# exosports/transit

Hardware: AMD Instinct MI355X
Metric: wavenumber-points*layers/sec (CH4 2-4um emission spectrum) (higher is better)
Workload: dtype f64; 1 GPU; BASELINE configs[1]: CH4-demo-shaped emission: 2500-5000 cm-1 @1 cm-1, wnosamp 2160, CH4 lines, eclipse, 5 angles, H2-H2 CIA; n_wn=2501, n_layers=100, layers_needed=81, n_lines=1000000, parallelism=one GPU

## Files before the change

transit_amd/csrc/hip/trx_api.hip:

```cpp
#include <hip/hip_runtime.h>
#include <rccl/rccl.h>
#include <dlfcn.h>
#include <functional>

#include <algorithm>
#include <chrono>
#include <cmath>
#include <cstdio>
#include <cstdlib>
#include <cstring>
#include <atomic>
#include <condition_variable>
#include <memory>
#include <mutex>
#include <string>
#include <thread>
#include <vector>

#include "transit_hip.h"
#include "trx_kernels.hip.h"
#include "trx_walk.hip.h"
#include "trx_rows.hip.h"
#include "trx_tail.hip.h"
#include "trx_lanes.hip.h"
// ... 9 lines not shown
  void release() { if (p) { (void)hipFree(p); p = nullptr; bytes = 0; } }
  template <class T> T *as() const { return (T *)p; }
};

struct DevView {
  void *p = nullptr;
  template <class T> T *as() const { return (T *)p; }
};

}

struct trx_handle {
  int device = 0;
  hipStream_t stream = nullptr, stream2 = nullptr;
  hipStream_t stream4 = nullptr;
  std::vector<hipEvent_t> ev_ac, ev_cb;
  hipEvent_t ev_walk1 = nullptr;
  hipEvent_t ev_inputs = nullptr, ev_cia = nullptr, ev_join = nullptr, ev_run_a = nullptr, ev_run_b = nullptr;
  std::string err;

  double wn_i = 0, wn_d = 0, odwn = 0; int64_t nwn = 0, nown = 0, lo = 0, hi = 0, nsh = 0; int osamp = 1;
  int niso = 0, nmol = 0;
  std::vector<double> iso_mass, iso_ratio, mol_mass, mol_radius, mol_pol;
  std::vector<double> pair_csd, pair_sqrt;
  std::vector<int32_t> iso_imol, mol_is_h2;
  std::vector<double> iso_wmin, iso_wmax;
  int ndop = 0, nlor = 0;
  std::vector<double> adop, alor;
  std::vector<int32_t> psizeT; bool psize_mono = false;
  std::vector<double> dopthr;
  std::vector<double> lorthr;
  std::vector<int> guess_dop, guess_lor, guess_a0, guess_a1;
  std::vector<long> guess_npre;
  std::vector<double> iso_sqrtm;
  std::vector<double> dens_over_m;
  std::vector<int32_t> psize; std::vector<long long> poff; int64_t tab_n = 0;
  DevBuf d_adop, d_dopthr, d_e2tab, d_psize, d_poff, d_tab, d_tabT, d_poffT, d_gimod, d_gidiv;
  float *tab = nullptr; const float *tabT = nullptr; const long long *poffT = nullptr;
  DevBuf d_tabW, d_walkprof; const float *tabW = nullptr; bool tabw_ok = false;
  DevBuf d_tabW32, d_wp32; const float *tabW32 = nullptr; unsigned slab32 = 0;
  long long row_m8_from = 768;
  std::vector<std::pair<double, double>> recip_ok;
  bool shard_frames = true;
  bool cia_window = true;
  bool cia_sums = true;
  bool cia_segments = true;
  bool two_queues = true;
  bool tail_direct = true;
  bool ray_tail = true;
  bool packed_walk = true; int packed_max_layers = 10;
  bool no_binrec = false;
  int xcd_map = 1;
  bool lanes_walk = true, lanes_force = false; int max_gcount = 0; DevBuf d_linebase, d_rinfo;
  bool no_row_copy = false, no_rows32 = false;
  bool row_staging = true;
  int64_t nlines = 0, ngroups = 0, nadd = 0, ninrange = 0;
  DevBuf d_lgroup, d_wavn, d_elow, d_gf, d_iso, d_inr, d_gfirst, d_gcount, d_giown, d_giso, d_gwavn, d_gblock, d_cntge, d_cntsub;
  int sub_f = 1;
  LinesDev L{};
  HostBuf<double> h_gwavn; std::vector<int32_t> h_gblock; HostBuf<int32_t> h_cntge, h_gfirst, h_gcount;
  void *comm = nullptr; int nranks = 1, rank = 0;
  bool windowed() const { return lo > 0 || hi < nwn; }
  DevBuf d_cand, d_candrec; int64_t ncand = -1;
  DevBuf d_kmax;
  int kmax_parity = 0, kmax_nr = 0; bool kmax_clean = false;
  DevBuf d_walk, d_wbase, d_part[2];
  std::vector<int32_t> h_wbase; int nwaves = 0, ngw = 0; bool walk_ok = false;
  bool walk_temp_ok = true;
  struct Plan { bool built = false; DevBuf blo, bhi, off, binw, binrec; int64_t records = 0; };
  Plan plan[4];
  struct Cia { int nspec; int mol[2]; std::vector<double> wn, temp, cs, zt, uw, ruw, rh, wf, wb; DevBuf d_wn, d_temp, d_cs, d_zt, d_uw, d_ruw, d_rh, d_wf, d_wb; };
  std::vector<Cia> cia;
  DevBuf d_cia_ws;
  int ws_nr = 0, ws_chunk = 0;
  DevBuf d_SG, d_idop8, d_sticky, d_part3;
  DevBuf d_in; void *h_in = nullptr; size_t h_in_bytes = 0; const double *h_in_dev = nullptr;
  DevBuf d_pm_f64, d_pm_i32;
  DevBuf d_xf;
  DevBuf d_small; DevView d_flags, d_status, d_counters; void *h_small = nullptr; size_t h_small_bytes = 0;
  DevBuf d_e, d_ecs, d_er, d_tau, d_last, d_intens, d_spec, d_acc, d_geom;
  bool has_grid = false; long og_nmol = 0, og_ntemp = 0, og_nlayer = 0, og_nwave = 0;
  std::vector<double> og_temp; std::vector<int32_t> og_molidx; DevBuf d_og_o, d_og_layer, d_og_itemp, d_iso_mx, d_pm, d_kmaxpm;
  trx_stats stats{};
  std::vector<double> run_f64, run_geom, run_ipv; std::vector<int32_t> run_i32;
  int hint_layers = 0;
  DevBuf d_e_saved; std::vector<uint8_t> saved;
  void *h_spec = nullptr; size_t h_spec_bytes = 0;
  void *h_spec_dev = nullptr, *h_small_dev = nullptr;
  void *h_tailblk = nullptr, *h_tailblk_dev = nullptr; size_t h_tailblk_bytes = 0;
};

namespace {

struct LogSink { trx_log_fn fn = nullptr; void *user = nullptr; int max_level = 0; };
LogSink &log_sink() { static LogSink s; return s; }
void log_msg(int level, const std::string &msg)
{
  const LogSink s = log_sink();
  if (s.fn && level <= s.max_level) s.fn(level, msg.c_str(), s.user);
}

struct StageTimer {
  std::chrono::steady_clock::time_point t = std::chrono::steady_clock::now();
  void lap(const char *what) {
    const auto n = std::chrono::steady_clock::now();
    if (log_sink().fn && log_sink().max_level >= TRX_LOG_DEBUG) {
// ... 77 lines not shown
  logspace((double)s->lmin, (double)s->lmax, nl, h->alor);
  h->psize.assign((size_t)nd * nl, 0); h->poff.assign((size_t)nd * nl, 0);
  const double dwn = s->wn_d / s->osamp;
  int64_t total = 0, bins = 0;
  for (int i = 0; i < nd; i++)
    for (int j = 0; j < nl; j++) {
      const size_t k = (size_t)i * nl + j;
      if (h->adop[i] * 10.0 < h->alor[j] && i != 0) {
        h->psize[k] = h->psize[k - nl]; h->poff[k] = h->poff[k - nl];
        continue;
      }
      const float dop = (float)h->adop[i], lor = (float)h->alor[j];
      double big = dop; if (big < lor) big = lor;
      const double wv = big * s->timesalpha;
      int nv = 2 * (long)(wv / dwn + 0.5) + 1;
      if (nv < 2) nv = 3;
      if (nv > 2 * (int)s->nown) nv = 2 * (int)s->nown + 1;
      if (nv < 0) return fail(h, TRX_E_ARG, "negative Voigt profile size");
      ProfileJob J{};
      J.off = total; J.nv = nv; J.alphaL = lor; J.alphaD = dop;
      J.half = dwn * (long)(nv / 2);
      const bool quick = nv > 99999;
      double step = 2.0 * J.half / (nv - 1);
      int npts = 50; double sub = J.alphaD / (npts - 1);
      if (step < sub || quick) { sub = step; J.regime = quick ? 0 : 1; J.m = 1; }
      else {
        npts = (int)(step / sub) + 1;
        if (npts & 1) npts++;
        J.m = npts; J.regime = 2;
        const long long tot = (long long)nv * npts + 1;
        if (tot > 2000000000LL) return fail(h, TRX_E_UNSUPPORTED, "Voigt sub-sampling exceeds int range");
        sub = 2.0 * J.half / (double)(tot - 1);
      }
      J.sub = sub; J.first_bin = bins;
      jobs.push_back(J);
      h->psize[k] = nv / 2; h->poff[k] = total;
      total += nv; bins += nv;
    }
  h->tab_n = total;
  return TRX_OK;
}

void test_switches(trx_handle *h)
{
  h->no_row_copy = std::getenv("TRX_NO_ROW_COPY") != nullptr;
  h->no_rows32 = std::getenv("TRX_NO_ROWS32") != nullptr;
  h->row_staging = !std::getenv("TRX_NO_ROW_STAGING");
  if (const char *v = std::getenv("TRX_ROWS_M8_FROM")) h->row_m8_from = std::atoll(v);
  h->packed_walk = !std::getenv("TRX_NO_PACKED_WALK");
  if (const char *v = std::getenv("TRX_PACKED_MAX_LAYERS")) h->packed_max_layers = std::max(1, std::min(32, std::atoi(v)));
  if (const char *e = std::getenv("TRX_XCD_MAP")) h->xcd_map = std::atoi(e);
  h->no_binrec = std::getenv("TRX_NO_BINREC") != nullptr;
  if (const char *e = std::getenv("TRX_LANES_WALK")) { h->lanes_walk = std::atoi(e) != 0; h->lanes_force = std::atoi(e) == 2; }
  if (const char *e = std::getenv("TRX_RAY_TAIL")) h->ray_tail = std::atoi(e) != 0;
  if (const char *e = std::getenv("TRX_CIA_SUMS")) h->cia_sums = std::atoi(e) != 0;
  if (const char *e = std::getenv("TRX_CIA_SEGMENTS")) h->cia_segments = std::atoi(e) != 0;
  if (const char *e = std::getenv("TRX_TWO_QUEUES")) h->two_queues = std::atoi(e) != 0;
  if (const char *e = std::getenv("TRX_TAIL_DIRECT")) h->tail_direct = std::atoi(e) != 0;
  if (const char *e = std::getenv("TRX_CIA_WINDOW")) h->cia_window = std::atoi(e) != 0;
  if (const char *e = std::getenv("TRX_SHARD_FRAMES")) h->shard_frames = std::atoi(e) != 0;
}

int build_table(trx_handle *h, const trx_static *s)
{
  std::vector<ProfileJob> jobs;
  int rc = plan_table(h, s, jobs);
  if (rc) return rc;
  double coef[64]; long double fact = 1.0L;
  for (int n = 0; n < 64; n++) { if (n > 0) fact *= (long double)n; coef[n] = (double)(1.0L / (fact * (long double)(2 * n + 1))); }
  HIPCHK(h, hipMemcpyToSymbolAsync(HIP_SYMBOL(c_voigt_coef), coef, sizeof(coef), 0, hipMemcpyHostToDevice, h->stream));
  DevBuf d_jobs;
  if ((rc = upload(h, d_jobs, jobs))) return rc;
  const size_t tab_alloc = (size_t)h->tab_n + 2 * kTabPad + (size_t)kWalkMaxFrame * (size_t)std::min<int64_t>(s->osamp, 1 << 21) + kRowTail;
  if ((rc = ensure(h, h->d_tab, sizeof(float) * tab_alloc))) return rc;
  HIPCHK(h, hipMemsetAsync(h->d_tab.p, 0, sizeof(float) * tab_alloc, h->stream));
  h->tab = h->d_tab.as<float>() + kTabPad;
  std::vector<int32_t> ps32(h->psize.begin(), h->psize.end());
  if ((rc = upload(h, h->d_psize, ps32))) return rc;
  if ((rc = upload(h, h->d_poff, h->poff))) return rc;
  if ((rc = upload(h, h->d_adop, h->adop))) return rc;
  {
    const int nd = s->ndop;
    std::vector<double> thr((size_t)nd + 1);
    thr[0] = -HUGE_VAL; thr[nd] = HUGE_VAL;
    auto idx = [&](double v) { return nearest_index(h->adop.data(), v, 0, nd); };
    for (int k = 1; k < nd; k++) {
      uint64_t a, b; double x;
      std::memcpy(&a, &h->adop[k - 1], 8); std::memcpy(&b, &h->adop[k], 8);
      while (b - a > 1) {
        const uint64_t m = a + (b - a) / 2;
        std::memcpy(&x, &m, 8);
        if (idx(x) >= k) b = m; else a = m;
      }
      std::memcpy(&thr[k], &b, 8);
      if (idx(thr[k]) != k || idx(std::nextafter(thr[k], 0.0)) != k - 1)
        return fail(h, TRX_E_ARG, "Doppler-width grid is not strictly increasing");
    }
    if ((rc = upload(h, h->d_dopthr, thr))) return rc;
    h->dopthr = thr;
    {
      const int nl = s->nlor;
      std::vector<double> lt((size_t)nl + 1);
      lt[0] = -HUGE_VAL; lt[nl] = HUGE_VAL;
      auto lidx = [&](double v) { return nearest_index(h->alor.data(), v, 0, nl); };
      bool ok = true;
      for (int k = 1; k < nl && ok; k++) {
// ... 59 lines not shown
                         d_joffT.as<long long>() + j0, h->tab, h->d_tabT.as<float>() + kTabPad, s->osamp, 0);
    }
    HIPCHK(h, hipStreamSynchronize(h->stream));
    h->tabT = h->d_tabT.as<float>() + kTabPad; h->poffT = h->d_poffT.as<long long>();
  }
  {
    std::vector<long long> joffW(jobs.size());
    long long totW = 0;
    for (size_t j = 0; j < jobs.size(); j++) {
      int front, stride; walk_row_layout((jobs[j].nv - 1) / s->osamp + 1, front, stride);
      joffW[j] = totW; totW += (long long)s->osamp * stride;
    }
    test_switches(h);
    h->tabw_ok = 4 * (totW + 2 * (long long)kTabPad) < (1LL << 32) && !h->no_row_copy;
    if (h->tabw_ok) {
      std::vector<WalkProfile> desc((size_t)s->ndop * s->nlor);
      size_t j = 0;
      for (int i = 0; i < s->ndop; i++)
        for (int k = 0; k < s->nlor; k++) {
          const size_t e = (size_t)i * s->nlor + k;
          if (h->adop[i] * 10.0 < h->alor[k] && i != 0) { desc[e] = desc[e - s->nlor]; continue; }
          const long long ps = h->psize[e], K = (2 * ps) / s->osamp + 1;
          int front, stride; walk_row_layout((int)K, front, stride);
          desc[e].centre4 = (uint32_t)(4 * (joffW[j++] + front + ps / s->osamp));
          desc[e].rowb = (int32_t)(4 * stride);
          desc[e].psr = (int32_t)(ps % s->osamp);
          desc[e].ps = (int32_t)ps;
        }
      DevBuf d_joffW;
      if ((rc = upload(h, d_joffW, joffW)) || (rc = upload(h, h->d_walkprof, desc))) return rc;
      if ((rc = ensure(h, h->d_tabW, sizeof(float) * ((size_t)totW + 2 * kTabPad)))) return rc;
      HIPCHK(h, hipMemsetAsync(h->d_tabW.p, 0, sizeof(float) * ((size_t)totW + 2 * kTabPad), h->stream));
      for (size_t j0 = 0; j0 < jobs.size(); j0 += 32768) {
        const int nj = (int)std::min<size_t>(32768, jobs.size() - j0);
        hipLaunchKernelGGL(k_table_phase_major, dim3(32, nj), dim3(256), 0, h->stream, d_jobs.as<ProfileJob>() + j0,
                           d_joffW.as<long long>() + j0, h->tab, h->d_tabW.as<float>() + kTabPad, s->osamp, 1);
      }
      {
        std::vector<long long> joff32(jobs.size(), -1);
        std::vector<uint32_t> c32((size_t)s->ndop * s->nlor, 0xffffffffu);
        long long nq = 0; size_t jj = 0;
        for (int i = 0; i < s->ndop; i++)
          for (int k = 0; k < s->nlor; k++) {
            const size_t e = (size_t)i * s->nlor + k;
            if (h->adop[i] * 10.0 < h->alor[k] && i != 0) { c32[e] = c32[e - s->nlor]; continue; }
            const long long ps = h->psize[e], K = (2 * ps) / s->osamp + 1;
            if (K <= 8) { joff32[jj] = 8 * nq; c32[e] = (uint32_t)(32 * nq); nq++; }
            jj++;
          }
        const long long tot32 = nq * 8 * (long long)s->osamp;
        if (nq > 0 && 32 * nq < (1LL << 24) && s->osamp < (1 << 24) && 4 * tot32 < (1LL << 32) && !h->no_rows32) {
          DevBuf d_joff32;
          if ((rc = upload(h, d_joff32, joff32)) || (rc = upload(h, h->d_wp32, c32))) return rc;
          if ((rc = ensure(h, h->d_tabW32, sizeof(float) * (size_t)tot32))) return rc;
          for (size_t j0 = 0; j0 < jobs.size(); j0 += 32768) {
            const int nj = (int)std::min<size_t>(32768, jobs.size() - j0);
            hipLaunchKernelGGL(k_table_rows32, dim3(16, nj), dim3(256), 0, h->stream, d_jobs.as<ProfileJob>() + j0,
                               d_joffW.as<long long>() + j0, d_joff32.as<long long>() + j0, h->d_tabW.as<float>() + kTabPad, h->d_tabW32.as<float>(), s->osamp, 8 * nq);
          }
          h->slab32 = (unsigned)(32 * nq);
          HIPCHK(h, hipStreamSynchronize(h->stream));
          h->tabW32 = h->d_tabW32.as<float>();
        }
      }
      HIPCHK(h, hipStreamSynchronize(h->stream));
      h->tabW = h->d_tabW.as<float>() + kTabPad;
    }
  }
  HIPCHK(h, hipGetLastError());
  HIPCHK(h, hipEventRecord(e1, h->stream));
  HIPCHK(h, hipStreamSynchronize(h->stream));
  float ms = 0; HIPCHK(h, hipEventElapsedTime(&ms, e0, e1));
  (void)hipEventDestroy(e0); (void)hipEventDestroy(e1);
  h->stats.ms_create_table = ms;
  h->stats.table_floats = h->tab_n;
  return TRX_OK;
}

int prepare_lines(trx_handle *h, const trx_static *s)
{
  const int64_t n = s->nlines;
  StageTimer T;
  const int nth = create_threads();
  const double wn0 = s->wn_i, odwn = s->wn_d / s->osamp;
  const double own_last = wn0 + (double)(s->nown - 1) * odwn;
  if (n > 2000000000LL) return fail(h, TRX_E_UNSUPPORTED, "more than 2^31 lines per handle");
  const double *elow = s->elow, *gf = s->gf;
  int rc_raw = TRX_OK;
  std::thread raw_up([&]() {
    (void)hipSetDevice(h->device);
    if ((rc_raw = upload_raw(h, h->d_elow, elow, (size_t)n)) || (rc_raw = upload_raw(h, h->d_gf, gf, (size_t)n)) ||
        (rc_raw = upload_raw(h, h->d_iso, s->isoid, (size_t)n))) return;
  });
  struct Joiner { std::thread &t; ~Joiner() { if (t.joinable()) t.join(); } } raw_join{raw_up};
  HostBuf<double> wavn; wavn.alloc((size_t)n);
  HostBuf<uint8_t> inr; inr.alloc((size_t)n);
  {
    std::vector<int64_t> cnt((size_t)nth + 1, 0); std::vector<int> bad((size_t)nth + 1, 0);
    parallel_parts(n, nth, [&](int t, int64_t i0, int64_t i1) {
      int64_t c = 0;
      for (int64_t i = i0; i < i1; i++) {
        if (s->isoid[i] < 0 || s->isoid[i] >= s->niso) { bad[t] = 1; continue; }
        wavn[i] = 1.0 / (s->wl_um[i] * kTliWfct);
        inr[i] = !(wavn[i] < wn0 || wavn[i] > own_last);
        c += inr[i];
      }
      cnt[t] = c;
// ... 617 lines not shown
  if (!M.permol) { h->stats.walk_steps++; h->stats.walk_records += pl->records; h->stats.walk_record_lanes += pl->records * nc; }
  const size_t pbytes = sizeof(double) * kWalkLayers * (size_t)std::max<int64_t>(pl->records, 1);
  if (part.bytes < pbytes) {
    HIPCHK(h, hipStreamSynchronize(st));
    HIPCHK(h, hipStreamSynchronize(h->stream4));
    if ((rc = ensure(h, part, pbytes))) return rc;
  }
  if (ev_reuse) HIPCHK(h, hipStreamWaitEvent(st, ev_reuse, 0));
  WalkArgs A{};
  A.lines = h->d_walk.as<WalkLine>(); A.rinfo = h->d_rinfo.as<RangeInfo>(); A.gfirst = h->d_gfirst.as<int32_t>(); A.gcount = h->d_gcount.as<int32_t>();
  A.gblock = h->d_gblock.as<int32_t>(); A.P = P;
  A.niso = h->niso; A.nlor = h->nlor; A.ndop = h->ndop; A.osamp = h->osamp; A.lo = h->lo; A.hi = h->hi;
  A.r_top = r_top; A.nc = nc; A.Y = Y; A.wcut = d_wcut; A.kmax = M.d_kmax; A.ethresh = M.ethresh;
  A.nmx = M.nmx; A.iso_mx = M.d_iso_mx; A.permol = M.permol; A.sticky_idop = M.d_sticky;
  A.dthr = h->d_dopthr.as<double>(); A.e2tab = h->d_e2tab.as<double>();
  A.psize = h->d_psize.as<int32_t>(); A.poff = h->d_poff.as<long long>();
  A.table = h->tab; A.zero_index = h->tab_n;
  A.tabw = h->tabW; A.walkprof = h->d_walkprof.as<WalkProfile>();
  A.tabw32 = h->tabW32; A.wp32 = h->tabW32 ? h->d_wp32.as<uint32_t>() : nullptr; A.slab32 = h->slab32;
  A.xcd_map = h->xcd_map & 2;
  A.part = part.as<double>(); A.counters = M.prof ? h->d_counters.as<unsigned long long>() : nullptr;
  A.flags = h->d_flags.as<int>(); A.last = M.skip_done ? h->d_last.as<int>() : nullptr; A.eager = M.eager;
  unsigned nw = (unsigned)h->nwaves;
  A.nseg = 0;
  if (h->windowed() && h->niso <= kWalkSegs && nw > 0) {
    const int Rc = nb / 2 - 1;
    const long long klo = std::max<long long>(0, h->lo - Rc - 1), khi = std::min<long long>(h->nwn - 1, h->hi - 1 + Rc);
    int cum = 0, ns = 0;
    for (int b = 0; b < h->niso; b++) {
      const int gb0 = h->h_gblock[b], gb1 = h->h_gblock[b + 1];
      if (gb0 == gb1) continue;
      const int32_t *cg = &h->h_cntge[(size_t)b * (h->nwn + 1)];
      const int ga = cg[khi + 1], gz = h->lo - Rc - 1 <= 0 ? gb1 - gb0 : cg[klo];
      const int wa = h->h_wbase[b] + ga / h->ngw, wz = h->h_wbase[b] + (gz + h->ngw - 1) / h->ngw;
      if (wz <= wa) continue;
      A.seg_w0[ns] = wa; A.seg_cum[ns] = cum; cum += wz - wa; ns++;
    }
    A.seg_cum[ns] = cum; A.nseg = ns;
    nw = (unsigned)cum;
    if (ns == 0) { A.nseg = 1; A.seg_w0[0] = 0; A.seg_cum[0] = 0; A.seg_cum[1] = 0; }
  }
  const bool lanes_prod = nw > 0 && A.tabw != nullptr && nb >= 8 && nc <= kLanesMaxLayers && h->lanes_walk &&
                          h->max_gcount <= kLanesMaxGroup && (h->ngroups >= 8 * h->nwn || h->lanes_force);
  const bool packed_prod = !lanes_prod && nw > 0 && A.tabw != nullptr && nc <= h->packed_max_layers && h->packed_walk;
  const bool lanes = lanes_prod && !M.prof, packed = packed_prod && !M.prof;
  const int form_prod = lanes_prod ? 1 : packed_prod ? 2 : 0, form = lanes ? 1 : packed ? 2 : 0;
  if (form_out) *form_out = form_prod;
  if (!M.permol) { h->stats.walk_form_steps[form_prod]++; h->stats.walk_form_layers[form_prod] += nc; h->stats.walk_form_record_lanes[form_prod] += pl->records * nc; }
  if (sp && sp->begin(form == 1 ? Spans::kWalkLanes : form == 2 ? Spans::kWalkPacked : Spans::kWalk, st)) return fail(h, TRX_E_HIP, "event");
  if (lanes) {
    LanesExtra X{h->d_linebase.as<double>()};
    A.xcd_map = h->xcd_map & 1;
    if (log_sink().fn && log_sink().max_level >= TRX_LOG_DEBUG)
      log_msg(TRX_LOG_DEBUG, "walk: lanes = lines, " + std::to_string(nc) + " layers, " + std::to_string(nb) + "-bin frames");
    const dim3 grid((nw + kLanesWaves - 1) / kLanesWaves), block(64 * kLanesWaves);
    const size_t lds = lanes_lds_bytes(nc, h->ndop);
    if (nb == 8) hipLaunchKernelGGL((k_line_walk_lanes<8, 5>), grid, block, lds, st, A, X);
    else         hipLaunchKernelGGL((k_line_walk_lanes<16, 2>), grid, block, lds, st, A, X);
  }
  else if (packed) {
    const int S = 64 / nc;
    const unsigned pw = (nw + (unsigned)S - 1) / (unsigned)S;
    const dim3 grid((pw + kWalkWaves - 1) / kWalkWaves), block(64 * kWalkWaves);
    if (nb <= 4)      hipLaunchKernelGGL(k_line_walk_packed<4>, grid, block, 0, st, A, S);
    else if (nb == 8) hipLaunchKernelGGL(k_line_walk_packed<8>, grid, block, 0, st, A, S);
    else              hipLaunchKernelGGL(k_line_walk_packed<16>, grid, block, 0, st, A, S);
  }
  else if (nw > 0) {
    const bool per_bin = M.prof || (nb >= kWalkRowsFrom && A.tabw == nullptr);
    if (nb == 2) launch_walk<2>(A, per_bin, nw, st);
    else if (nb == 4) launch_walk<4>(A, per_bin, nw, st);
    else if (nb == 8) launch_walk<8>(A, per_bin, nw, st);
    else launch_walk<16>(A, per_bin, nw, st);
  }
  if (sp && sp->end(st)) return fail(h, TRX_E_HIP, "event");
  PendingCombine pc;
  pc.valid = true; pc.sc = st_comb ? st_comb : st; pc.st_walk = st; pc.cross = st_comb != nullptr && ev_walk != nullptr;
  pc.ev_walk = ev_walk; pc.ev_done = ev_done;
  if (pc.cross) HIPCHK(h, hipEventRecord(ev_walk, st));
  CombineArgs &C = pc.C;
  C.P = P; C.niso = h->niso; C.gblock = h->d_gblock.as<int32_t>(); C.lo = h->lo; C.nsh = h->nsh; C.r_top = r_top; C.nc = nc;
  C.nmx = M.nmx; C.iso_mx = M.d_iso_mx; C.part = part.as<double>(); C.e = M.d_e;
  C.flags = h->d_flags.as<int>(); C.last = A.last; C.eager = M.eager;
  if (defer) { *defer = pc; return TRX_OK; }
  return launch_combine(h, pc, sp);
}

int sweep_chunk(trx_handle *h, const LayerDev &Y, const double *d_wcut, const int32_t *psmax,
                int r_top, int nc, int nc_max, const SweepMode &M, Spans *sp)
{
  hipStream_t st = M.st ? M.st : h->stream;
  const int niso = h->niso; const int64_t nsh = h->nsh;
  const int ntiles = (int)((nsh + kTileBins - 1) / kTileBins);
  double *d_SG = h->d_SG.as<double>();
  uint8_t *d_idop8 = h->d_idop8.as<uint8_t>();
  SweepWindow Wn{};
  Wn.windowed = h->windowed() ? 1 : 0; Wn.osamp = h->osamp; Wn.lo = h->lo; Wn.hi = h->hi; Wn.nwn = h->nwn;
  long long seg_lines = 0;
  for (int b = 0; b < niso; b++) {
    const int gb0 = h->h_gblock[b], gb1 = h->h_gblock[b + 1];
    if (gb0 == gb1) continue;
    int ga = gb0, gz = gb1;
    if (h->windowed()) {
      long long psm = 0;
      for (int c = 0; c < nc; c++) psm = std::max<long long>(psm, psmax[(size_t)(r_top - c) * niso + b]);
      const long long lo_f = (long long)h->osamp * h->lo - psm;
      long long klo = lo_f > 0 ? lo_f / h->osamp : 0;
      long long khi = ((long long)h->osamp * (h->hi - 1) + psm) / h->osamp;
      if (khi > h->nwn - 1) khi = h->nwn - 1;
      const int32_t *cg = &h->h_cntge[(size_t)b * (h->nwn + 1)];
      ga = gb0 + cg[khi + 1]; gz = gb0 + cg[klo];
// ... 1368 lines not shown
```

transit_amd/csrc/hip/trx_lanes.hip.h:

```cpp
#pragma once
#include "trx_walk.hip.h"

namespace trx {

constexpr int kLanesWaves = 2;
constexpr int kLanesBatch = 32;
constexpr int kLanesMaxGroup = 16;
constexpr int kLanesMaxLayers = 32;
constexpr int kLanesLayK = 12;
constexpr int kLanesBases = 4;
constexpr int kLanesRows = kLanesBatch + 2;

struct LanesExtra {
  const double *wbase;
};

__host__ __device__ inline int lanes_at_doubles(int ne) { return ((kLanesRows * ne / 2) + 1) & ~1; }
__host__ __device__ inline int lanes_wave_doubles(int nc) { const int ne = (nc + 1) & ~1; return kLanesRows * ne + lanes_at_doubles(ne) + kLanesLayK * ne + kLanesBases * ne + kLanesBatch / 2; }
__host__ __device__ inline size_t lanes_lds_bytes(int nc, int ndop) { return (size_t)kLanesWaves * 8 * (size_t)lanes_wave_doubles(nc) + 8 * (size_t)(ndop + 1); }

__device__ __forceinline__ double wave_shl1(double v)
{
  const int lo = __builtin_amdgcn_update_dpp(0, __double2loint(v), 0x130, 0xF, 0xF, true);
  const int hi = __builtin_amdgcn_update_dpp(0, __double2hiint(v), 0x130, 0xF, 0xF, true);
  return __hiloint2double(hi, lo);
}

template <int NB, int D>
__global__ __launch_bounds__(64 * kLanesWaves)
void k_line_walk_lanes(WalkArgs A, LanesExtra X)
{
  constexpr int Rc = NB / 2 - 1, NS = NB / 2, LPL = 2, BL = kLanesBatch;
  static_assert(NB == 8 || NB == 16, "frames of 8 or 16 bins");
  if (!A.eager && A.flags[0] == 0) return;
  __shared__ double s_e2[64];
  extern __shared__ double s_dyn[];
  double *s_thr = s_dyn + (size_t)kLanesWaves * lanes_wave_doubles(A.nc);
  const double e2_mine = threadIdx.x < 64 ? A.e2tab[threadIdx.x] : 0.0;
  const int wv = __builtin_amdgcn_readfirstlane(threadIdx.x >> 6), lane = threadIdx.x & 63;
  const int nc = A.nc, ne = (nc + 1) & ~1;
  double *s_kk = s_dyn + (size_t)wv * lanes_wave_doubles(nc);
  uint32_t *s_at = (uint32_t *)(s_kk + kLanesRows * ne);
  double (*LK)[kLanesLayK] = (double (*)[kLanesLayK])(s_kk + kLanesRows * ne + lanes_at_doubles(ne));
  double *s_E0 = s_kk + kLanesRows * ne + lanes_at_doubles(ne) + kLanesLayK * ne;
  int *s_cellr = (int *)(s_E0 + kLanesBases * ne);

  const int nlaunch = A.nseg > 0 ? A.seg_cum[A.nseg] : A.P.nwaves;
  int w = (A.xcd_map ? xcd_block(blockIdx.x, gridDim.x) : (int)blockIdx.x) * kLanesWaves + wv;
  bool have = w < nlaunch;
  if (have && A.nseg > 0) {
    int sgm = 0;
    while (sgm + 1 < A.nseg && w >= A.seg_cum[sgm + 1]) sgm++;
    w = A.seg_w0[sgm] + (w - A.seg_cum[sgm]);
  }
  have = have && w < A.P.nwaves;
  int r_b = 0, l0 = 0, l1 = 0, blo = 0, bhi = -1, cell0 = 0; long long rec0 = 0; double wavn0 = 0.0;
  if (have) {
    const RangeInfo RI = A.rinfo[w];
    r_b = RI.b; l0 = RI.l0; l1 = RI.l1; wavn0 = RI.wavn0; cell0 = RI.cell0;
    blo = A.P.blo[w]; bhi = A.P.bhi[w]; rec0 = A.P.off[w];
  }
  for (int i = threadIdx.x; i <= A.ndop; i += 64 * kLanesWaves) s_thr[i] = A.dthr[i];
  if (threadIdx.x < 64) s_e2[threadIdx.x] = e2_mine;
  struct LayerScalars { double ad, ct, f, dens, kmax, wcut; int il, idst, idop0; } pre{};
  if (have && lane < ne) {
    const int cl = min(lane, nc - 1);
    const int r = A.r_top - cl, ri = r * A.niso + r_b;
    pre.ad = A.Y.alphad[ri]; pre.il = A.Y.ilor[ri]; pre.idst = A.sticky_idop[ri];
    pre.ct = A.Y.negc_over_t[r]; pre.f = A.Y.strength_f[ri]; pre.dens = A.permol ? 1.0 : A.Y.density[ri];
    pre.kmax = A.kmax[(long long)r * A.nmx + (A.nmx == 1 ? 0 : A.iso_mx[r_b])]; pre.wcut = A.wcut[ri]; pre.idop0 = A.Y.idop0[ri];
  }
  bool open = have && bhi >= blo;
  if (open && A.last) {
    bool o = false;
    for (int j = blo + lane; j <= bhi; j += 64) o |= A.last[j - A.lo] < 0;
    open = __ballot(o) != 0ull;
  }
  __syncthreads();
  if (!open) return;

  const int li = lane >> 1, part = lane & 1;
  const bool valid = li < nc;
  const int lic = valid ? li : 0;
  const bool r32 = NB == 8 && A.tabw32 != nullptr;
  const char *tabw_base = r32 ? (const char *)A.tabw32 : (const char *)A.tabw - 4 * (Rc + 1);
  const unsigned part_off = 4u * NS * (unsigned)part;
  const double *s_kk_lane = s_kk + lic; const uint32_t *s_at_lane = s_at + lic;
  double acc[NS];
#pragma unroll
  for (int k = 0; k < NS; k++) acc[k] = 0.0;
  int jc = cell0;
  auto flush = [&](int k, double v, bool mine) {
    const int j = jc - Rc + part * NS + k;
    if (valid && mine && j >= blo && j <= bhi) A.part[(rec0 + (j - blo)) * kWalkLayers + li] = v;
  };
  auto fill_zero = [&](int ja, int jb) {
    ja = max(ja, blo); jb = min(jb, bhi);
    if (valid && part == 0) for (int j = ja; j <= jb; j++) A.part[(rec0 + (j - blo)) * kWalkLayers + li] = 0.0;
  };
  auto shift_to = [&](int cell) {
    int sh = jc - cell;
    if (sh >= NB) {
#pragma unroll
      for (int k = 0; k < NS; k++) { flush(k, acc[k], true); acc[k] = 0.0; }
      fill_zero(cell + Rc + 2, jc - Rc - 1);
      jc = cell;
    } else {
      for (; sh > 0; sh--) {
        flush(NS - 1, acc[NS - 1], part == LPL - 1);
        const double carry = dpp_f64<0xB1>(acc[NS - 1]);
#pragma unroll
        for (int k = NS - 1; k > 0; k--) acc[k] = acc[k - 1];
        acc[0] = part == 1 ? carry : 0.0;
        jc--;
      }
    }
  };

  struct alignas(16) Row { float v[NS]; };
  double bk_kk[2][D]; Row bk_row[2][D];
  int bn[2] = {0, 0}, bcell[2] = {0, 0};
#pragma unroll
  for (int s = 0; s < 2; s++)
#pragma unroll
    for (int u = 0; u < D; u++) {
      bk_kk[s][u] = 0.0;
#pragma unroll
      for (int k = 0; k < NS; k++) bk_row[s][u].v[k] = 0.f;
    }
  auto consume = [&](auto SET) {
    constexpr int s = decltype(SET)::value;
    if (bn[s] != 0 && bcell[s] != jc) shift_to(bcell[s]);
#pragma unroll
    for (int u = 0; u < D; u++)
#pragma unroll
      for (int k = 0; k < NS; k++) acc[k] = __builtin_fma(bk_kk[s][u], (double)bk_row[s][u].v[k], acc[k]);
  };

  if (lane < ne) { s_kk[BL * ne + lane] = 0.0; s_at[BL * ne + lane] = 0u; s_at[(BL + 1) * ne + lane] = 0u; }

  if (lane < ne) {
    double *K = LK[lane];
    K[0] = pre.ct; K[1] = pre.f; K[2] = pre.dens;
    K[3] = A.ethresh * pre.kmax; K[4] = pre.wcut; K[5] = pre.ad;
    const int cur = index_from(s_thr, pre.ad * wavn0, pre.idop0);
    const WalkProfile wc_ = A.walkprof[cur * A.nlor + pre.il], ws_ = A.walkprof[pre.idst * A.nlor + pre.il];
    K[6] = s_thr[cur];
    int *KI = (int *)(K + 7);
    KI[0] = cur; KI[1] = pre.il;
    KI[2] = r32 ? (int)A.wp32[cur * A.nlor + pre.il] : (int)wc_.centre4 + 4; KI[3] = wc_.rowb; KI[4] = wc_.psr; KI[5] = 0;
    KI[6] = r32 ? (int)A.wp32[pre.idst * A.nlor + pre.il] : (int)ws_.centre4 + 4; KI[7] = ws_.rowb; KI[8] = ws_.psr; KI[9] = pre.idst;
  }

  struct Lines { double wavn, elow, gf, wb; int meta, cell; };
  auto geometry = [&](int l_at, int &lg) { const int left = l1 - l_at; lg = left > 16 ? 5 : left > 8 ? 4 : 3; };
  auto fetch = [&](int l_at) -> Lines {
    int lg; geometry(l_at, lg);
    const int BLx = 1 << lg, t1 = lane & (BLx - 1);
    const bool in0 = t1 < min(BLx, l1 - l_at);
    const int at = l_at + (in0 ? t1 : 0);
    const WalkLine *lp = A.lines + at;
    Lines b; b.wavn = lp->wavn; b.elow = lp->elow; b.gf = lp->gf; b.meta = in0 ? lp->meta : 0; b.cell = lp->cell; b.wb = X.wbase[at];
    return b;
  };
  double c24 = 0x1.5555555555555p-5;
  asm volatile("" : "+v"(c24));
  Lines cur = fetch(l0);
  int e0_prev = -1;
  __builtin_amdgcn_wave_barrier();
  bn[1] = 0; bcell[1] = cell0;
#pragma unroll
  for (int u = 0; u < D; u++) {
    bk_kk[1][u] = s_kk_lane[BL * ne];
    __builtin_memcpy(&bk_row[1][u], tabw_base + (s_at_lane[BL * ne] + part_off + 32u * u), sizeof(Row));
  }

  for (int l = l0; l < l1; ) {
    int lg; geometry(l, lg);
    const int BLx = 1 << lg, nsets = 64 >> lg;
    const int t1 = lane & (BLx - 1), h1 = lane >> lg;
    const int n0 = min(BLx, l1 - l);
    const bool in0 = t1 < n0;
    const double wavn = cur.wavn, elow = cur.elow, wb = cur.wb;
    const int meta = cur.meta, v_cell = cur.cell;
    const unsigned lowm = (unsigned)((1ull << BLx) - 1ull);
    const unsigned ends = (unsigned)__ballot(in0 && (meta & 2)) & lowm;
    const int n = ends ? 32 - __builtin_clz(ends) : n0;
    const bool in = t1 < n;
    const double gf = in ? cur.gf : 0.0;
    const bool is_anchor = in && (meta & 1);
    const unsigned amask = (unsigned)__ballot(is_anchor) & lowm;
    const int nanch = __builtin_popcount(amask);
    const int rank = __builtin_popcount(amask & (unsigned)((1ull << t1) - 1ull));
    const int prev_cell = __builtin_amdgcn_update_dpp(0, v_cell, 0x138, 0xF, 0xF, false);
    unsigned bstart_r = 0u;
    for (unsigned m = (unsigned)__ballot(is_anchor && t1 > 0 && prev_cell != v_cell) & lowm; m; m &= m - 1u)
      bstart_r |= 1u << __builtin_popcount(amask & ((1u << __builtin_ctz(m)) - 1u));
    if (is_anchor && h1 == 0) s_cellr[rank] = v_cell;
    const int rowk = (is_anchor ? rank : BL + 1) * ne;
    int len = 1;
    { const unsigned e = ends >> t1; if (is_anchor && e) len = __builtin_ctz(e) + 1; }
    int kmax_len = 1;
    while (__any(kmax_len < len)) kmax_len++;
    const double m1 = len > 1 ? 1.0 : 0.0;
    const int imod = meta >> 3;
    const unsigned leaders = ((unsigned)__ballot(in && ((meta & 4) || t1 == 0))) & lowm;
    const int nlead = __builtin_popcount(leaders);
    const bool e0_tab = nlead <= kLanesBases;
    const int bid = __builtin_popcount(leaders & (unsigned)((2ull << t1) - 1ull)) - 1;
    if (e0_tab) {
      unsigned lm = leaders; int j = 0;
      if (e0_prev >= 0 && !(__builtin_amdgcn_readfirstlane(meta) & 4)) {
        if (e0_prev != 0 && lane < ne) s_E0[lane] = s_E0[e0_prev * ne + lane];
        lm &= lm - 1u; j = 1;
      }
      for (; j < nlead; j++) {
        const int tl = __builtin_ctz(lm); lm &= lm - 1u;
        const double wbj = readlane_f64(wb, tl);
        if (lane < ne) s_E0[j * ne + lane] = exp_neg(LK[lane][0] * wbj, s_e2);
      }
      e0_prev = nlead - 1;
    } else e0_prev = -1;
    bool step = false;
    { const double wl = readlane_f64(wavn, n - 1); if (lane < ne) step = LK[lane][5] * wl < LK[lane][6]; }
    const bool slow = __any(step);
    __builtin_amdgcn_wave_barrier();
    auto layer = [&](int c2, auto E0TAB, auto SLOW, auto CLAMP) {
      const int c = decltype(CLAMP)::value ? min(c2 + h1, ne - 1) : c2 + h1;
      double *K = LK[c];
      struct alignas(16) D2 { double a, b; }; struct alignas(16) I4 { int x, y, z, w; };
      const D2 k01 = *(const D2 *)(K + 0), k23 = *(const D2 *)(K + 2);
      const double ct = k01.a, f = k01.b, dens = k23.a, lim = k23.b, wc = K[4];
      I4 pc = *(const I4 *)(K + 8); const I4 ps = *(const I4 *)(K + 10);
      const double e1 = exp_neg(ct * elow, s_e2, c24);
      const double t0 = ct * wb;
      double E0;
      if constexpr (decltype(E0TAB)::value) E0 = s_E0[bid * ne + c]; else E0 = exp_neg(t0, s_e2, c24);
      const double q = __builtin_fma(-E0, exp_small(__builtin_fma(ct, wavn, -t0), c24), 1.0);
      const double s = gf * e1 * q;
      double pk = s;
      if (kmax_len > 1) {
        double sh = wave_shl1(s);
        pk = __builtin_fma(sh, m1, pk);
        for (int k = 2; k < kmax_len; k++) {
          sh = wave_shl1(sh);
          pk += k < len ? sh : 0.0;
        }
      }
      const double pkf = pk * f;
      const double kk = pkf < lim ? 0.0 : pkf * dens;
      if constexpr (decltype(SLOW)::value) {
        const double v = K[5] * wavn;
        int *KI = (int *)(K + 7);
        const int cur_i = KI[0];
        int idx = cur_i; double th = K[6];
        while (__any(in && v < th)) { if (in && v < th) { idx--; th = s_thr[idx]; } }
        if (idx != cur_i) { const WalkProfile wp = A.walkprof[idx * A.nlor + KI[1]]; pc.x = r32 ? (int)A.wp32[idx * A.nlor + KI[1]] : (int)wp.centre4 + 4; pc.y = wp.rowb; pc.z = wp.psr; }
        const int ncur = __shfl(idx, (n - 1) + (h1 << lg), 64);
        __builtin_amdgcn_wave_barrier();
        if (t1 == 0 && c2 + h1 < ne && ncur != cur_i) {
          const WalkProfile wp = A.walkprof[ncur * A.nlor + KI[1]];
          K[6] = s_thr[ncur]; KI[0] = ncur; KI[2] = r32 ? (int)A.wp32[ncur * A.nlor + KI[1]] : (int)wp.centre4 + 4; KI[3] = wp.rowb; KI[4] = wp.psr;
        }
      }
      const bool own = wavn >= wc;
      const int c4p = own ? pc.x : ps.x, rb = own ? pc.y : ps.y, psr = own ? pc.z : ps.z;
      const int d = psr - imod, sgn = d >> 31;
      const unsigned rowsel = (unsigned)(d + (sgn & A.osamp));
      const unsigned at = r32 ? (unsigned)c4p + __umul24((unsigned)imod, A.slab32)
                              : __umul24(rowsel, (unsigned)rb) + (unsigned)(c4p + (sgn << 2));
      s_kk[rowk + c] = kk; s_at[rowk + c] = at;
    };
    using T = std::true_type; using F = std::false_type;
    if (slow)             for (int c2 = 0; c2 < ne; c2 += nsets) layer(c2, F{}, T{}, T{});
    else if (!e0_tab)     for (int c2 = 0; c2 < ne; c2 += nsets) layer(c2, F{}, F{}, T{});
    else if (nsets != 2)  for (int c2 = 0; c2 < ne; c2 += nsets) layer(c2, T{}, F{}, T{});
    else                  for (int c2 = 0; c2 < ne; c2 += 2)     layer(c2, T{}, F{}, F{});
    __builtin_amdgcn_wave_barrier();

    const int l_next = l + n;
    if (l_next < l1) cur = fetch(l_next);

    const int c_rank = s_cellr[lane & (BL - 1)];
    int j = 0;
    auto block_end = [&](int a) {
      const unsigned nxt = bstart_r >> a >> 1;
      return nxt ? min(nanch, a + 1 + __builtin_ctz(nxt)) : nanch;
    };
    int nblk = 0;
    for (int a = 0; a < nanch; ) { const int e = block_end(a); nblk += (e - a + D - 1) / D; a = e; }
    bool pad = nblk & 1;
    auto produce = [&](auto SET, bool empty) {
      constexpr int s = decltype(SET)::value;
      const int cnt = empty ? 0 : min(D, block_end(j) - j);
      bcell[s] = __builtin_amdgcn_readlane(c_rank, min(j, BL - 1)); bn[s] = cnt;
#pragma unroll
      for (int u = 0; u < D; u++) {
        const int row = (u < cnt ? j + u : BL) * ne;
        bk_kk[s][u] = s_kk_lane[row];
        __builtin_memcpy(&bk_row[s][u], tabw_base + (s_at_lane[row] + part_off), sizeof(Row));
      }
      j += cnt;
    };
    int it = (nblk + 1) >> 1;
    do {
      produce(std::integral_constant<int, 0>{}, pad); pad = false;
      consume(std::integral_constant<int, 1>{});
      produce(std::integral_constant<int, 1>{}, false);
      consume(std::integral_constant<int, 0>{});
    } while (--it > 0);
    __builtin_amdgcn_wave_barrier();
    l = l_next;
  }
  consume(std::integral_constant<int, 1>{});
#pragma unroll
  for (int k = 0; k < NS; k++) flush(k, acc[k], true);
  fill_zero(blo, jc - Rc - 1);
}

}
```

Before: 833.3 million wavenumber-points*layers/s.

## Split each layer's frame bins across up to four lanes in lanes walk

The lanes line-walk kernel is generalised from two lanes per layer to a template parameter P (2–4) chosen from the layer count, so each lane accumulates fewer frame bins and more of the wave's 64 lanes are busy when there are few layers. Carries between lane parts use a P-dependent DPP shuffle, and the LDS layout switches to an odd stride (nc|1), which looks intended to avoid bank conflicts. Row loads shrink to 4*NS bytes with smaller alignment, and the rows32 table gains zeroed slack so the reads stay in bounds. The risks are more per-lane overhead on the shift/flush logic, unaligned narrower loads, and extra template instantiations.

```diff
diff --git a/transit_amd/csrc/hip/trx_api.hip b/transit_amd/csrc/hip/trx_api.hip
--- a/transit_amd/csrc/hip/trx_api.hip
+++ b/transit_amd/csrc/hip/trx_api.hip
@@ -85,6 +85,7 @@
   bool no_binrec = false;
   int xcd_map = 1;
   bool lanes_walk = true, lanes_force = false; int max_gcount = 0; DevBuf d_linebase, d_rinfo;
+  int lanes_parts_most = 4;
   bool no_row_copy = false, no_rows32 = false;
   bool row_staging = true;
   int64_t nlines = 0, ngroups = 0, nadd = 0, ninrange = 0;
@@ -268,6 +269,7 @@
   if (const char *e = std::getenv("TRX_XCD_MAP")) h->xcd_map = std::atoi(e);
   h->no_binrec = std::getenv("TRX_NO_BINREC") != nullptr;
   if (const char *e = std::getenv("TRX_LANES_WALK")) { h->lanes_walk = std::atoi(e) != 0; h->lanes_force = std::atoi(e) == 2; }
+  if (const char *e = std::getenv("TRX_LANES_PARTS")) h->lanes_parts_most = std::max(2, std::min(4, std::atoi(e)));
   if (const char *e = std::getenv("TRX_RAY_TAIL")) h->ray_tail = std::atoi(e) != 0;
   if (const char *e = std::getenv("TRX_CIA_SUMS")) h->cia_sums = std::atoi(e) != 0;
   if (const char *e = std::getenv("TRX_CIA_SEGMENTS")) h->cia_segments = std::atoi(e) != 0;
@@ -433,7 +435,8 @@
         if (nq > 0 && 32 * nq < (1LL << 24) && s->osamp < (1 << 24) && 4 * tot32 < (1LL << 32) && !h->no_rows32) {
           DevBuf d_joff32;
           if ((rc = upload(h, d_joff32, joff32)) || (rc = upload(h, h->d_wp32, c32))) return rc;
-          if ((rc = ensure(h, h->d_tabW32, sizeof(float) * (size_t)tot32))) return rc;
+          if ((rc = ensure(h, h->d_tabW32, sizeof(float) * ((size_t)tot32 + kLanesRowSlack)))) return rc;
+          HIPCHK(h, hipMemsetAsync(h->d_tabW32.as<float>() + tot32, 0, sizeof(float) * kLanesRowSlack, h->stream));
           for (size_t j0 = 0; j0 < jobs.size(); j0 += 32768) {
             const int nj = (int)std::min<size_t>(32768, jobs.size() - j0);
             hipLaunchKernelGGL(k_table_rows32, dim3(16, nj), dim3(256), 0, h->stream, d_jobs.as<ProfileJob>() + j0,
@@ -1157,11 +1160,20 @@
     LanesExtra X{h->d_linebase.as<double>()};
     A.xcd_map = h->xcd_map & 1;
     if (log_sink().fn && log_sink().max_level >= TRX_LOG_DEBUG)
-      log_msg(TRX_LOG_DEBUG, "walk: lanes = lines, " + std::to_string(nc) + " layers, " + std::to_string(nb) + "-bin frames");
+      log_msg(TRX_LOG_DEBUG, "walk: lanes = lines, " + std::to_string(nc) + " layers, " + std::to_string(nb) + "-bin frames, " +
+                             std::to_string(lanes_parts(nc, h->lanes_parts_most)) + " lanes per layer");
     const dim3 grid((nw + kLanesWaves - 1) / kLanesWaves), block(64 * kLanesWaves);
     const size_t lds = lanes_lds_bytes(nc, h->ndop);
-    if (nb == 8) hipLaunchKernelGGL((k_line_walk_lanes<8, 5>), grid, block, lds, st, A, X);
-    else         hipLaunchKernelGGL((k_line_walk_lanes<16, 2>), grid, block, lds, st, A, X);
+    const int parts = lanes_parts(nc, h->lanes_parts_most);
+    if (nb == 8) {
+      if (parts == 4)      hipLaunchKernelGGL((k_line_walk_lanes<8, 5, 4>), grid, block, lds, st, A, X);
+      else if (parts == 3) hipLaunchKernelGGL((k_line_walk_lanes<8, 5, 3>), grid, block, lds, st, A, X);
+      else                 hipLaunchKernelGGL((k_line_walk_lanes<8, 5, 2>), grid, block, lds, st, A, X);
+    } else {
+      if (parts == 4)      hipLaunchKernelGGL((k_line_walk_lanes<16, 2, 4>), grid, block, lds, st, A, X);
+      else if (parts == 3) hipLaunchKernelGGL((k_line_walk_lanes<16, 2, 3>), grid, block, lds, st, A, X);
+      else                 hipLaunchKernelGGL((k_line_walk_lanes<16, 2, 2>), grid, block, lds, st, A, X);
+    }
   }
   else if (packed) {
     const int S = 64 / nc;
diff --git a/transit_amd/csrc/hip/trx_lanes.hip.h b/transit_amd/csrc/hip/trx_lanes.hip.h
--- a/transit_amd/csrc/hip/trx_lanes.hip.h
+++ b/transit_amd/csrc/hip/trx_lanes.hip.h
@@ -9,14 +9,18 @@
 constexpr int kLanesMaxLayers = 32;
 constexpr int kLanesLayK = 12;
 constexpr int kLanesBases = 4;
+constexpr int kLanesRowSlack = 8;
 constexpr int kLanesRows = kLanesBatch + 2;
 
 struct LanesExtra {
   const double *wbase;
 };
 
-__host__ __device__ inline int lanes_at_doubles(int ne) { return ((kLanesRows * ne / 2) + 1) & ~1; }
-__host__ __device__ inline int lanes_wave_doubles(int nc) { const int ne = (nc + 1) & ~1; return kLanesRows * ne + lanes_at_doubles(ne) + kLanesLayK * ne + kLanesBases * ne + kLanesBatch / 2; }
+__host__ __device__ inline int lanes_parts(int nc, int most = 4) { return min(most, nc <= 16 ? 4 : nc <= 21 ? 3 : 2); }
+
+__host__ __device__ inline int lanes_stride(int nc) { return nc | 1; }
+__host__ __device__ inline int lanes_at_doubles(int ns) { return ((kLanesRows * ns + 1) / 2 + 1) & ~1; }
+__host__ __device__ inline int lanes_wave_doubles(int nc) { const int ns = lanes_stride(nc); return kLanesRows * ns + lanes_at_doubles(ns) + kLanesLayK * nc + kLanesBases * ns + kLanesBatch / 2; }
 __host__ __device__ inline size_t lanes_lds_bytes(int nc, int ndop) { return (size_t)kLanesWaves * 8 * (size_t)lanes_wave_doubles(nc) + 8 * (size_t)(ndop + 1); }
 
 __device__ __forceinline__ double wave_shl1(double v)
@@ -26,24 +30,31 @@
   return __hiloint2double(hi, lo);
 }
 
-template <int NB, int D>
+template <int P>
+__device__ __forceinline__ double carry_up(double v)
+{
+  return dpp_f64<P == 2 ? 0xB1 : P == 4 ? 0x111 : 0x138>(v);
+}
+
+template <int NB, int D, int P>
 __global__ __launch_bounds__(64 * kLanesWaves)
 void k_line_walk_lanes(WalkArgs A, LanesExtra X)
 {
-  constexpr int Rc = NB / 2 - 1, NS = NB / 2, LPL = 2, BL = kLanesBatch;
+  constexpr int Rc = NB / 2 - 1, NS = (NB + P - 1) / P, NL = NB - (P - 1) * NS, BL = kLanesBatch;
   static_assert(NB == 8 || NB == 16, "frames of 8 or 16 bins");
+  static_assert(P >= 2 && P <= 4 && NL >= 1 && NL <= NS, "2 to 4 lanes per layer");
   if (!A.eager && A.flags[0] == 0) return;
   __shared__ double s_e2[64];
   extern __shared__ double s_dyn[];
   double *s_thr = s_dyn + (size_t)kLanesWaves * lanes_wave_doubles(A.nc);
   const double e2_mine = threadIdx.x < 64 ? A.e2tab[threadIdx.x] : 0.0;
   const int wv = __builtin_amdgcn_readfirstlane(threadIdx.x >> 6), lane = threadIdx.x & 63;
-  const int nc = A.nc, ne = (nc + 1) & ~1;
+  const int nc = A.nc, ns = lanes_stride(nc);
   double *s_kk = s_dyn + (size_t)wv * lanes_wave_doubles(nc);
-  uint32_t *s_at = (uint32_t *)(s_kk + kLanesRows * ne);
-  double (*LK)[kLanesLayK] = (double (*)[kLanesLayK])(s_kk + kLanesRows * ne + lanes_at_doubles(ne));
-  double *s_E0 = s_kk + kLanesRows * ne + lanes_at_doubles(ne) + kLanesLayK * ne;
-  int *s_cellr = (int *)(s_E0 + kLanesBases * ne);
+  uint32_t *s_at = (uint32_t *)(s_kk + kLanesRows * ns);
+  double (*LK)[kLanesLayK] = (double (*)[kLanesLayK])(s_kk + kLanesRows * ns + lanes_at_doubles(ns));
+  double *s_E0 = s_kk + kLanesRows * ns + lanes_at_doubles(ns) + kLanesLayK * nc;
+  int *s_cellr = (int *)(s_E0 + kLanesBases * ns);
 
   const int nlaunch = A.nseg > 0 ? A.seg_cum[A.nseg] : A.P.nwaves;
   int w = (A.xcd_map ? xcd_block(blockIdx.x, gridDim.x) : (int)blockIdx.x) * kLanesWaves + wv;
@@ -63,9 +74,8 @@
   for (int i = threadIdx.x; i <= A.ndop; i += 64 * kLanesWaves) s_thr[i] = A.dthr[i];
   if (threadIdx.x < 64) s_e2[threadIdx.x] = e2_mine;
   struct LayerScalars { double ad, ct, f, dens, kmax, wcut; int il, idst, idop0; } pre{};
-  if (have && lane < ne) {
-    const int cl = min(lane, nc - 1);
-    const int r = A.r_top - cl, ri = r * A.niso + r_b;
+  if (have && lane < nc) {
+    const int r = A.r_top - lane, ri = r * A.niso + r_b;
     pre.ad = A.Y.alphad[ri]; pre.il = A.Y.ilor[ri]; pre.idst = A.sticky_idop[ri];
     pre.ct = A.Y.negc_over_t[r]; pre.f = A.Y.strength_f[ri]; pre.dens = A.permol ? 1.0 : A.Y.density[ri];
     pre.kmax = A.kmax[(long long)r * A.nmx + (A.nmx == 1 ? 0 : A.iso_mx[r_b])]; pre.wcut = A.wcut[ri]; pre.idop0 = A.Y.idop0[ri];
@@ -79,7 +89,7 @@
   __syncthreads();
   if (!open) return;
 
-  const int li = lane >> 1, part = lane & 1;
+  const int li = lane / P, part = lane - li * P;
   const bool valid = li < nc;
   const int lic = valid ? li : 0;
   const bool r32 = NB == 8 && A.tabw32 != nullptr;
@@ -102,22 +112,22 @@
     int sh = jc - cell;
     if (sh >= NB) {
 #pragma unroll
-      for (int k = 0; k < NS; k++) { flush(k, acc[k], true); acc[k] = 0.0; }
+      for (int k = 0; k < NS; k++) { flush(k, acc[k], k < NL || part != P - 1); acc[k] = 0.0; }
       fill_zero(cell + Rc + 2, jc - Rc - 1);
       jc = cell;
     } else {
       for (; sh > 0; sh--) {
-        flush(NS - 1, acc[NS - 1], part == LPL - 1);
-        const double carry = dpp_f64<0xB1>(acc[NS - 1]);
+        flush(NL - 1, acc[NL - 1], part == P - 1);
+        const double carry = carry_up<P>(acc[NS - 1]);
 #pragma unroll
         for (int k = NS - 1; k > 0; k--) acc[k] = acc[k - 1];
-        acc[0] = part == 1 ? carry : 0.0;
+        acc[0] = part != 0 ? carry : 0.0;
         jc--;
       }
     }
   };
 
-  struct alignas(16) Row { float v[NS]; };
+  struct alignas(NS % 4 == 0 ? 16 : NS % 2 == 0 ? 8 : 4) Row { float v[NS]; };
   double bk_kk[2][D]; Row bk_row[2][D];
   int bn[2] = {0, 0}, bcell[2] = {0, 0};
 #pragma unroll
@@ -137,9 +147,9 @@
       for (int k = 0; k < NS; k++) acc[k] = __builtin_fma(bk_kk[s][u], (double)bk_row[s][u].v[k], acc[k]);
   };
 
-  if (lane < ne) { s_kk[BL * ne + lane] = 0.0; s_at[BL * ne + lane] = 0u; s_at[(BL + 1) * ne + lane] = 0u; }
-
-  if (lane < ne) {
+  if (lane < nc) { s_kk[BL * ns + lane] = 0.0; s_at[BL * ns + lane] = 0u; s_at[(BL + 1) * ns + lane] = 0u; }
+
+  if (lane < nc) {
     double *K = LK[lane];
     K[0] = pre.ct; K[1] = pre.f; K[2] = pre.dens;
     K[3] = A.ethresh * pre.kmax; K[4] = pre.wcut; K[5] = pre.ad;
@@ -171,12 +181,14 @@
   bn[1] = 0; bcell[1] = cell0;
 #pragma unroll
   for (int u = 0; u < D; u++) {
-    bk_kk[1][u] = s_kk_lane[BL * ne];
-    __builtin_memcpy(&bk_row[1][u], tabw_base + (s_at_lane[BL * ne] + part_off + 32u * u), sizeof(Row));
+    bk_kk[1][u] = s_kk_lane[BL * ns];
+    __builtin_memcpy(&bk_row[1][u], tabw_base + (s_at_lane[BL * ns] + part_off + 32u * u), 4 * NS);
   }
 
   for (int l = l0; l < l1; ) {
     int lg; geometry(l, lg);
+    int ncb = nc;
+    asm volatile("" : "+s"(ncb));
     const int BLx = 1 << lg, nsets = 64 >> lg;
     const int t1 = lane & (BLx - 1), h1 = lane >> lg;
     const int n0 = min(BLx, l1 - l);
@@ -197,7 +209,7 @@
     for (unsigned m = (unsigned)__ballot(is_anchor && t1 > 0 && prev_cell != v_cell) & lowm; m; m &= m - 1u)
       bstart_r |= 1u << __builtin_popcount(amask & ((1u << __builtin_ctz(m)) - 1u));
     if (is_anchor && h1 == 0) s_cellr[rank] = v_cell;
-    const int rowk = (is_anchor ? rank : BL + 1) * ne;
+    const int rowk = (is_anchor ? rank : BL + 1) * ns;
     int len = 1;
     { const unsigned e = ends >> t1; if (is_anchor && e) len = __builtin_ctz(e) + 1; }
     int kmax_len = 1;
@@ -211,22 +223,22 @@
     if (e0_tab) {
       unsigned lm = leaders; int j = 0;
       if (e0_prev >= 0 && !(__builtin_amdgcn_readfirstlane(meta) & 4)) {
-        if (e0_prev != 0 && lane < ne) s_E0[lane] = s_E0[e0_prev * ne + lane];
+        if (e0_prev != 0 && lane < ncb) s_E0[lane] = s_E0[e0_prev * ns + lane];
         lm &= lm - 1u; j = 1;
       }
       for (; j < nlead; j++) {
         const int tl = __builtin_ctz(lm); lm &= lm - 1u;
         const double wbj = readlane_f64(wb, tl);
-        if (lane < ne) s_E0[j * ne + lane] = exp_neg(LK[lane][0] * wbj, s_e2);
+        if (lane < ncb) s_E0[j * ns + lane] = exp_neg(LK[lane][0] * wbj, s_e2);
       }
       e0_prev = nlead - 1;
     } else e0_prev = -1;
     bool step = false;
-    { const double wl = readlane_f64(wavn, n - 1); if (lane < ne) step = LK[lane][5] * wl < LK[lane][6]; }
+    { const double wl = readlane_f64(wavn, n - 1); if (lane < ncb) step = LK[lane][5] * wl < LK[lane][6]; }
     const bool slow = __any(step);
     __builtin_amdgcn_wave_barrier();
     auto layer = [&](int c2, auto E0TAB, auto SLOW, auto CLAMP) {
-      const int c = decltype(CLAMP)::value ? min(c2 + h1, ne - 1) : c2 + h1;
+      const int c = decltype(CLAMP)::value ? min(c2 + h1, nc - 1) : c2 + h1;
       double *K = LK[c];
       struct alignas(16) D2 { double a, b; }; struct alignas(16) I4 { int x, y, z, w; };
       const D2 k01 = *(const D2 *)(K + 0), k23 = *(const D2 *)(K + 2);
@@ -235,7 +247,7 @@
       const double e1 = exp_neg(ct * elow, s_e2, c24);
       const double t0 = ct * wb;
       double E0;
-      if constexpr (decltype(E0TAB)::value) E0 = s_E0[bid * ne + c]; else E0 = exp_neg(t0, s_e2, c24);
+      if constexpr (decltype(E0TAB)::value) E0 = s_E0[bid * ns + c]; else E0 = exp_neg(t0, s_e2, c24);
       const double q = __builtin_fma(-E0, exp_small(__builtin_fma(ct, wavn, -t0), c24), 1.0);
       const double s = gf * e1 * q;
       double pk = s;
@@ -258,7 +270,7 @@
         if (idx != cur_i) { const WalkProfile wp = A.walkprof[idx * A.nlor + KI[1]]; pc.x = r32 ? (int)A.wp32[idx * A.nlor + KI[1]] : (int)wp.centre4 + 4; pc.y = wp.rowb; pc.z = wp.psr; }
         const int ncur = __shfl(idx, (n - 1) + (h1 << lg), 64);
         __builtin_amdgcn_wave_barrier();
-        if (t1 == 0 && c2 + h1 < ne && ncur != cur_i) {
+        if (t1 == 0 && c2 + h1 < nc && ncur != cur_i) {
           const WalkProfile wp = A.walkprof[ncur * A.nlor + KI[1]];
           K[6] = s_thr[ncur]; KI[0] = ncur; KI[2] = r32 ? (int)A.wp32[ncur * A.nlor + KI[1]] : (int)wp.centre4 + 4; KI[3] = wp.rowb; KI[4] = wp.psr;
         }
@@ -272,10 +284,10 @@
       s_kk[rowk + c] = kk; s_at[rowk + c] = at;
     };
     using T = std::true_type; using F = std::false_type;
-    if (slow)             for (int c2 = 0; c2 < ne; c2 += nsets) layer(c2, F{}, T{}, T{});
-    else if (!e0_tab)     for (int c2 = 0; c2 < ne; c2 += nsets) layer(c2, F{}, F{}, T{});
-    else if (nsets != 2)  for (int c2 = 0; c2 < ne; c2 += nsets) layer(c2, T{}, F{}, T{});
-    else                  for (int c2 = 0; c2 < ne; c2 += 2)     layer(c2, T{}, F{}, F{});
+    if (slow)                       for (int c2 = 0; c2 < nc; c2 += nsets) layer(c2, F{}, T{}, T{});
+    else if (!e0_tab)               for (int c2 = 0; c2 < nc; c2 += nsets) layer(c2, F{}, F{}, T{});
+    else if (nsets != 2 || (nc & 1)) for (int c2 = 0; c2 < nc; c2 += nsets) layer(c2, T{}, F{}, T{});
+    else                            for (int c2 = 0; c2 < nc; c2 += 2)     layer(c2, T{}, F{}, F{});
     __builtin_amdgcn_wave_barrier();
 
     const int l_next = l + n;
@@ -296,9 +308,9 @@
       bcell[s] = __builtin_amdgcn_readlane(c_rank, min(j, BL - 1)); bn[s] = cnt;
 #pragma unroll
       for (int u = 0; u < D; u++) {
-        const int row = (u < cnt ? j + u : BL) * ne;
+        const int row = (u < cnt ? j + u : BL) * ns;
         bk_kk[s][u] = s_kk_lane[row];
-        __builtin_memcpy(&bk_row[s][u], tabw_base + (s_at_lane[row] + part_off), sizeof(Row));
+        __builtin_memcpy(&bk_row[s][u], tabw_base + (s_at_lane[row] + part_off), 4 * NS);
       }
       j += cnt;
     };
@@ -314,7 +326,7 @@
   }
   consume(std::integral_constant<int, 1>{});
 #pragma unroll
-  for (int k = 0; k < NS; k++) flush(k, acc[k], true);
+  for (int k = 0; k < NS; k++) flush(k, acc[k], k < NL || part != P - 1);
   fill_zero(blo, jc - Rc - 1);
 }
 
```

After: 856.9 million wavenumber-points*layers/s, median of 6. 2.8% higher.
